# gmh14/tssplat

Measured on AMD Instinct MI355X. Metric: tetrahedra/sec (energy fwd+bwd), higher is better.
Workload: dtype f32

## Files before the change

### include/tssplat_amd.h

```cpp
#ifndef TSSPLAT_AMD_H
#define TSSPLAT_AMD_H

#include <stdint.h>

#ifdef __cplusplus
extern "C" {
#endif

typedef struct tsamd_handle tsamd_handle;

typedef enum tsamd_status {
    TSAMD_OK = 0,
    TSAMD_ERR_INVALID_ARGUMENT = 1,
    TSAMD_ERR_BAD_MESH = 2,
    TSAMD_ERR_NO_DEVICE = 3,
    TSAMD_ERR_HIP = 4,
    TSAMD_ERR_IO = 5,
    TSAMD_ERR_TILING = 6,
    TSAMD_ERR_HOST_ONLY = 7
} tsamd_status;

typedef struct tsamd_options {
    int32_t struct_size;
    int32_t device;
// ... 11 lines not shown

typedef struct tsamd_plan_info {
    int64_t n_vertices, n_tets;
    int64_t n_tiles;
    int64_t n_components;
    int64_t total_slots;
    int64_t total_tile_vertices;
    int64_t shared_vertex_copies;
    int64_t finish_vertices;
    int64_t device_bytes;
    int32_t max_slots, max_tile_vertices, block_threads, lds_bytes;
    int32_t slots_per_thread;
    int32_t n_planes;
} tsamd_plan_info;

typedef struct tsamd_tile_view {
    int32_t n_slots, n_owned, s_pad, n_verts, n_excl;
    int64_t stage_off;
    int32_t n_rows;
    int32_t rec_base;
    const uint32_t *planes;
    const uint16_t *row_start;
    const int32_t *gvid;
    const int32_t *vdst;
    const int32_t *slot_tet;
    const float *rest;
} tsamd_tile_view;

const char *tsamd_last_error(void);
const char *tsamd_version(void);
#define TSAMD_ABI_VERSION 3
int32_t tsamd_abi_version(void);

int tsamd_create(const float *rest_xyz, int64_t n_vertices, const int32_t *tets, int64_t n_tets,
                 const tsamd_options *options, tsamd_handle **out);
int tsamd_create_from_veg(const char *path, const tsamd_options *options, tsamd_handle **out);
int tsamd_create_with_operator(const float *rest_xyz, int64_t n_vertices, const int32_t *tets, int64_t n_tets,
                               const int64_t *op_rowptr, const int32_t *op_col, const double *op_val,
                               const tsamd_options *options, tsamd_handle **out);
void tsamd_destroy(tsamd_handle *h);

int64_t tsamd_num_vertices(const tsamd_handle *h);
int64_t tsamd_num_tets(const tsamd_handle *h);
int tsamd_get_plan_info(const tsamd_handle *h, tsamd_plan_info *out);
int tsamd_get_tile(const tsamd_handle *h, int64_t tile, tsamd_tile_view *out);
int tsamd_get_finish_lists(const tsamd_handle *h, int64_t *n_finish, const int32_t **vid,
                           const int32_t **off, const int32_t **idx);
int tsamd_get_adjacency(const tsamd_handle *h, const int32_t **nbr);

int tsamd_forward(tsamd_handle *h, const float *x_dev, float c1, float c2, int order,
                  void *stream, float *energy_dev);
int tsamd_backward(tsamd_handle *h, const float *x_dev, const float *grad_out_dev, float c1, float c2,
                   int order, void *stream, float *grad_dev);
int tsamd_forward_backward(tsamd_handle *h, const float *x_dev, const float *grad_out_dev, float c1,
                           float c2, int order, void *stream, float *energy_dev, float *grad_dev);
int tsamd_evaluate_dev_coef(tsamd_handle *h, const float *x_dev, const float *grad_out_dev, const float *coef_dev,
                            int order, void *stream, float *energy_dev, float *grad_dev);
typedef struct tsamd_graph tsamd_graph;
int tsamd_graph_create(tsamd_handle *h, const float *x_dev, const float *grad_out_dev, int order, float *energy_dev,
// ... 101 lines not shown
```

### tssplat_amd/_capi.py

```python
from __future__ import annotations

import ctypes as C
import os

from . import _build

_lib = None


class TsamdError(RuntimeError):

    def __init__(self, code: int, message: str):
        super().__init__(f"tssplat_amd error {code}: {message}")
        self.code = code


class Options(C.Structure):
    _fields_ = [
        ("struct_size", C.c_int32),
        ("device", C.c_int32),
        ("lds_budget_bytes", C.c_int32),
        ("max_threads", C.c_int32),
        ("target_owned", C.c_int32),
        ("lane_search_sweeps", C.c_int32),
# ... 7 lines not shown


class PlanInfo(C.Structure):
    _fields_ = [
        ("n_vertices", C.c_int64), ("n_tets", C.c_int64), ("n_tiles", C.c_int64),
        ("n_components", C.c_int64), ("total_slots", C.c_int64), ("total_tile_vertices", C.c_int64),
        ("shared_vertex_copies", C.c_int64), ("finish_vertices", C.c_int64), ("device_bytes", C.c_int64),
        ("max_slots", C.c_int32), ("max_tile_vertices", C.c_int32), ("block_threads", C.c_int32),
        ("lds_bytes", C.c_int32), ("slots_per_thread", C.c_int32), ("n_planes", C.c_int32),
    ]

    def as_dict(self) -> dict:
        return {k: int(getattr(self, k)) for k, _ in self._fields_}


class TileView(C.Structure):
    _fields_ = [
        ("n_slots", C.c_int32), ("n_owned", C.c_int32), ("s_pad", C.c_int32), ("n_verts", C.c_int32),
        ("n_excl", C.c_int32), ("stage_off", C.c_int64), ("n_rows", C.c_int32), ("rec_base", C.c_int32),
        ("planes", C.POINTER(C.c_uint32)), ("row_start", C.POINTER(C.c_uint16)),
        ("gvid", C.POINTER(C.c_int32)), ("vdst", C.POINTER(C.c_int32)), ("slot_tet", C.POINTER(C.c_int32)), ("rest", C.POINTER(C.c_float)),
    ]


ABI_VERSION = 3

SIGNATURES = {
    "tsamd_last_error": (C.c_char_p, []),
    "tsamd_version": (C.c_char_p, []),
    "tsamd_abi_version": (C.c_int32, []),
    "tsamd_create": (C.c_int, [C.c_void_p, C.c_int64, C.c_void_p, C.c_int64, C.POINTER(Options), C.POINTER(C.c_void_p)]),
    "tsamd_create_with_operator": (C.c_int, [C.c_void_p, C.c_int64, C.c_void_p, C.c_int64, C.c_void_p, C.c_void_p, C.c_void_p,
                                             C.POINTER(Options), C.POINTER(C.c_void_p)]),
    "tsamd_create_from_veg": (C.c_int, [C.c_char_p, C.POINTER(Options), C.POINTER(C.c_void_p)]),
    "tsamd_destroy": (None, [C.c_void_p]),
    "tsamd_num_vertices": (C.c_int64, [C.c_void_p]),
    "tsamd_num_tets": (C.c_int64, [C.c_void_p]),
    "tsamd_get_plan_info": (C.c_int, [C.c_void_p, C.POINTER(PlanInfo)]),
    "tsamd_get_tile": (C.c_int, [C.c_void_p, C.c_int64, C.POINTER(TileView)]),
    "tsamd_get_finish_lists": (C.c_int, [C.c_void_p, C.POINTER(C.c_int64), C.POINTER(C.POINTER(C.c_int32)),
                                         C.POINTER(C.POINTER(C.c_int32)), C.POINTER(C.POINTER(C.c_int32))]),
    "tsamd_get_adjacency": (C.c_int, [C.c_void_p, C.POINTER(C.POINTER(C.c_int32))]),
    "tsamd_forward": (C.c_int, [C.c_void_p, C.c_void_p, C.c_float, C.c_float, C.c_int, C.c_void_p, C.c_void_p]),
    "tsamd_backward": (C.c_int, [C.c_void_p, C.c_void_p, C.c_void_p, C.c_float, C.c_float, C.c_int, C.c_void_p,
                                 C.c_void_p]),
    "tsamd_forward_backward": (C.c_int, [C.c_void_p, C.c_void_p, C.c_void_p, C.c_float, C.c_float, C.c_int,
                                         C.c_void_p, C.c_void_p, C.c_void_p]),
    "tsamd_evaluate_dev_coef": (C.c_int, [C.c_void_p, C.c_void_p, C.c_void_p, C.c_void_p, C.c_int, C.c_void_p, C.c_void_p,
                                          C.c_void_p]),
    "tsamd_graph_create": (C.c_int, [C.c_void_p, C.c_void_p, C.c_void_p, C.c_int, C.c_void_p, C.c_void_p, C.POINTER(C.c_void_p)]),
    "tsamd_graph_launch": (C.c_int, [C.c_void_p, C.c_float, C.c_float, C.c_void_p]),
    "tsamd_graph_launch_to": (C.c_int, [C.c_void_p, C.c_float, C.c_float, C.c_void_p, C.c_void_p, C.c_void_p]),
    "tsamd_graph_destroy": (None, [C.c_void_p]),
# ... 134 lines not shown
```

### tssplat_amd/csrc/capi.cpp

```cpp
#include "../../include/tssplat_amd.h"

#include <hip/hip_runtime_api.h>

#include <algorithm>
#include <cmath>
#include <cstdio>
#include <cstdlib>
#include <cstring>
#include <new>
#include <string>
#include <thread>
#include <vector>

#include "capi_common.h"
#include "kernels.h"
#include "plan.h"

namespace {

thread_local std::string g_err;

int fail(int code, const std::string &msg)
{
    g_err = msg;
// ... 323 lines not shown
    out->n_components = P.n_components;
    out->total_slots = P.total_slots;
    out->total_tile_vertices = P.total_tile_verts;
    out->shared_vertex_copies = P.n_stage;
    out->finish_vertices = int64_t(P.fin_vid.size());
    out->device_bytes = h->device_bytes;
    out->max_slots = P.max_slots;
    out->max_tile_vertices = P.max_verts;
    out->block_threads = P.block_threads;
    out->lds_bytes = P.lds_bytes;
    out->slots_per_thread = P.spt;
    out->n_planes = P.n_planes;
    return TSAMD_OK;
}

int tsamd_get_tile(const tsamd_handle *h, int64_t tile, tsamd_tile_view *out)
{
    if (!h || !out) return fail(TSAMD_ERR_INVALID_ARGUMENT, "null argument");
    const tsamd::Plan &P = h->plan;
    if (tile < 0 || tile >= int64_t(P.tiles.size())) return fail(TSAMD_ERR_INVALID_ARGUMENT, "tile out of range");
    const tsamd::TileDesc &d = P.tiles[size_t(tile)];
    out->n_slots = d.n_slots;
    out->n_owned = d.n_owned;
    out->s_pad = d.s_pad;
    out->n_verts = d.n_verts;
    out->n_excl = d.n_excl;
    out->stage_off = d.stage_off;
    out->n_rows = d.n_rows;
    out->rec_base = d.rec_base;
    out->planes = P.blob.data() + d.blob_off / 4;
// ... 254 lines not shown
```

### tssplat_amd/csrc/partition.cpp

```cpp
#include "partition.h"

#include <algorithm>
#include <cmath>

namespace tsamd {
namespace {

constexpr int kLloydIters = 12;
constexpr int kLloydFull = 4;
constexpr int kCandidates = 8;
constexpr int kImproveSweeps = 6;
constexpr int kConnectProbe = 512;
constexpr int64_t kMaxIncidence = int64_t(1) << 23;

inline int64_t copies(int64_t c) { return (c + kMaxRank - 1) / kMaxRank; }

struct Part {
    const Limits &lim;
    int64_t cnt = 0, nv = 0, k = 0;
    std::vector<int32_t> nb;
    std::vector<int32_t> lv;
    std::vector<double> x;
    std::vector<int32_t> part;
    std::vector<int64_t> owned, slots, verts;
    std::vector<int32_t> inc;
    std::vector<int32_t> mark, queue;
    int32_t stamp = 0;

    explicit Part(const Limits &l) : lim(l) {}

    int64_t cost(int64_t p) const { return kPartSlotWeight * slots[size_t(p)] + verts[size_t(p)]; }
    bool fits(int64_t p) const { return lim.fits(slots[size_t(p)], verts[size_t(p)]); }

    void seed(int32_t *idx, int64_t n, int64_t kk, int32_t &next)
    {
        if (kk <= 1) {
            for (int64_t i = 0; i < n; ++i) part[size_t(idx[i])] = next;
            ++next;
            return;
        }
        double lo[3], hi[3];
        for (int d = 0; d < 3; ++d) {
            lo[d] = std::numeric_limits<double>::max();
            hi[d] = -std::numeric_limits<double>::max();
        }
        for (int64_t i = 0; i < n; ++i)
// ... 147 lines not shown
                        pc[np] = pr;
                        nn[np++] = 0;
                    }
                    ++nn[j];
                }
                if (np == 0) continue;
                int j = 0;
                for (int i = 1; i < np; ++i)
                    if (nn[i] > nn[j] || (nn[i] == nn[j] && pc[i] < pc[j])) j = i;
                part[size_t(e)] = pc[j];
                --left;
            }
        }
    }

    void add_slot(int32_t p, int32_t e)
    {
        ++slots[size_t(p)];
        for (int a = 0; a < 4; ++a) {
            int32_t &c = inc[size_t(p) * size_t(nv) + size_t(lv[4 * size_t(e) + a])];
            if (c % kMaxRank == 0) ++verts[size_t(p)];
            ++c;
        }
    }
    void remove_slot(int32_t p, int32_t e)
    {
        --slots[size_t(p)];
        for (int a = 0; a < 4; ++a) {
            int32_t &c = inc[size_t(p) * size_t(nv) + size_t(lv[4 * size_t(e) + a])];
            --c;
            if (c % kMaxRank == 0) --verts[size_t(p)];
        }
    }
    void build_state()
    {
        owned.assign(size_t(k), 0);
        slots.assign(size_t(k), 0);
        verts.assign(size_t(k), 0);
        inc.assign(size_t(k) * size_t(nv), 0);
        for (int64_t q = 0; q < cnt; ++q) {
            const int32_t pq = part[size_t(q)];
            ++owned[size_t(pq)];
            add_slot(pq, int32_t(q));
            int32_t seen[4];
            int ns = 0;
            for (int f = 0; f < 4; ++f) {
                const int32_t r = nb[4 * size_t(q) + f];
                if (r < 0) continue;
                const int32_t pr = part[size_t(r)];
                if (pr == pq || std::find(seen, seen + ns, pr) != seen + ns) continue;
                seen[ns++] = pr;
                add_slot(pr, int32_t(q));
            }
        }
// ... 28 lines not shown
            if (q < 0 || part[size_t(q)] == A || !first_of(e, f)) continue;
            if (in_cell(q, A) == 1) out[n++] = q;
        }
        return n;
    }
    int entering(int32_t e, int32_t B, int32_t *out) const
    {
        int n = 0;
        for (int f = 0; f < 4; ++f) {
            const int32_t q = nb[4 * size_t(e) + f];
            if (q < 0 || part[size_t(q)] == B || !first_of(e, f)) continue;
            if (in_cell(q, B) == 0) out[n++] = q;
        }
        return n;
    }
    int64_t vert_delta(int32_t p, const int32_t *t, int n, int sign) const
    {
        int32_t vs[20], ds[20];
        int m = 0;
        for (int i = 0; i < n; ++i)
            for (int a = 0; a < 4; ++a) {
                const int32_t v = lv[4 * size_t(t[i]) + a];
                int j = int(std::find(vs, vs + m, v) - vs);
                if (j == m) {
                    vs[m] = v;
                    ds[m++] = 0;
                }
                ds[j] += sign;
            }
        int64_t d = 0;
        for (int j = 0; j < m; ++j) {
            const int32_t c = inc[size_t(p) * size_t(nv) + size_t(vs[j])];
            d += copies(c + ds[j]) - copies(c);
        }
        return d;
    }
    struct Move {
        int32_t e = -1, B = -1;
        int64_t dcost = 0, key = 0;
        int nl = 0, ne = 0;
        int32_t gone[5], en[4];
        int64_t dsA = 0, dvA = 0, dsB = 0, dvB = 0;
    };
    bool evaluate(int32_t e, int32_t B, Move &mv) const
    {
        const int32_t A = part[size_t(e)];
        mv.e = e;
        mv.B = B;
        mv.nl = leaving(e, A, mv.gone);
        mv.ne = entering(e, B, mv.en);
        mv.dsA = -mv.nl;
        mv.dsB = mv.ne;
        mv.dvB = vert_delta(B, mv.en, mv.ne, +1);
        if (!lim.fits(slots[size_t(B)] + mv.dsB, verts[size_t(B)] + mv.dvB)) return false;
        mv.dvA = vert_delta(A, mv.gone, mv.nl, -1);
        mv.dcost = kPartSlotWeight * (mv.dsA + mv.dsB) + mv.dvA + mv.dvB;
        return true;
    }
    void apply(const Move &mv)
    {
        const int32_t A = part[size_t(mv.e)];
        for (int i = 0; i < mv.nl; ++i) remove_slot(A, mv.gone[i]);
        for (int i = 0; i < mv.ne; ++i) add_slot(mv.B, mv.en[i]);
        part[size_t(mv.e)] = mv.B;
        --owned[size_t(A)];
        ++owned[size_t(mv.B)];
    }
    bool stays_connected(int32_t e)
    {
        const int32_t A = part[size_t(e)];
        int32_t want[4];
// ... 40 lines not shown
        for (int64_t A = 0; A < k; ++A) {
            if (fits(A)) continue;
            members.clear();
            for (int64_t e = 0; e < cnt; ++e)
                if (part[size_t(e)] == A) members.push_back(int32_t(e));
            while (!fits(A)) {
                if (owned[size_t(A)] <= 1) return false;
                Move best, mv;
                bool have = false;
                for (int32_t e : members) {
                    if (part[size_t(e)] != A) continue;
                    int32_t oc[4];
                    const int no = other_cells(e, oc);
                    for (int j = 0; j < no; ++j) {
                        if (!evaluate(e, oc[j], mv)) continue;
                        mv.key = mv.dcost + kPartSlotWeight * mv.dsA + mv.dvA;
                        if (have && mv.key >= best.key) continue;
                        if (!stays_connected(e)) break;
                        best = mv;
                        have = true;
                    }
                }
                if (!have) return false;
                apply(best);
            }
        }
        return true;
    }

    void improve()
    {
        for (int sweep = 0; sweep < kImproveSweeps; ++sweep) {
            int64_t moved = 0;
            for (int64_t e = 0; e < cnt; ++e) {
                const int32_t A = part[size_t(e)];
                if (owned[size_t(A)] <= 1) continue;
                int32_t oc[4];
                const int no = other_cells(int32_t(e), oc);
                Move best, mv;
                bool have = false;
                for (int j = 0; j < no; ++j) {
                    if (!evaluate(int32_t(e), oc[j], mv) || mv.dcost >= 0) continue;
                    if (have && mv.dcost >= best.dcost) continue;
                    best = mv;
                    have = true;
                }
                if (have && stays_connected(int32_t(e))) {
                    apply(best);
                    ++moved;
                }
            }
            if (moved == 0) break;
        }
    }
};

}

bool partition_component(const Mesh &M, const Limits &lim, const float *cen, const int32_t *ids, int64_t cnt,
                         int64_t k_first, int64_t k_last, Scratch &S, std::vector<std::vector<int32_t>> &parts,
                         int64_t &cost)
{
    parts.clear();
    cost = 0;
    k_first = std::max<int64_t>(2, k_first);
    k_last = std::min(k_last, cnt);
    if (k_first > k_last) return false;
    Part P(lim);
    P.cnt = cnt;
    P.nb.resize(4 * size_t(cnt));
    P.lv.resize(4 * size_t(cnt));
    P.x.resize(3 * size_t(cnt));
    const int32_t st = S.next();
    for (int64_t i = 0; i < cnt; ++i) {
        S.tet_stamp[size_t(ids[i])] = st;
        S.tet_slot[size_t(ids[i])] = int32_t(i);
    }
    for (int64_t i = 0; i < cnt; ++i) {
        const int64_t g = ids[i];
        for (int f = 0; f < 4; ++f) {
            const int32_t q = M.nbr[4 * g + f];
            P.nb[4 * size_t(i) + f] = q >= 0 && S.tet_stamp[size_t(q)] == st ? S.tet_slot[size_t(q)] : -1;
            const int32_t v = M.tets[4 * g + f];
            if (S.vert_stamp[size_t(v)] != st) {
                S.vert_stamp[size_t(v)] = st;
                S.vert_local[size_t(v)] = int32_t(P.nv++);
            }
            P.lv[4 * size_t(i) + f] = S.vert_local[size_t(v)];
        }
        for (int d = 0; d < 3; ++d) P.x[3 * size_t(i) + d] = cen[3 * size_t(g) + d];
    }
    if (k_last * P.nv > kMaxIncidence) return false;
    P.mark.assign(size_t(cnt), 0);
    std::vector<int32_t> idx(static_cast<size_t>(cnt));
    for (int64_t k = k_first; k <= k_last; ++k) {
        P.k = k;
        P.part.assign(size_t(cnt), 0);
        for (int64_t i = 0; i < cnt; ++i) idx[size_t(i)] = int32_t(i);
        int32_t next = 0;
        P.seed(idx.data(), cnt, k, next);
        P.lloyd();
        P.connect();
        P.build_state();
        if (!P.repair()) continue;
        P.improve();
        std::vector<int64_t> at(size_t(k), -1);
        for (int64_t p = 0; p < k; ++p)
            if (P.owned[size_t(p)] > 0) {
                at[size_t(p)] = int64_t(parts.size());
                parts.emplace_back();
                parts.back().reserve(size_t(P.owned[size_t(p)]));
                cost += P.cost(p);
            }
        for (int64_t i = 0; i < cnt; ++i) parts[size_t(at[size_t(P.part[size_t(i)])])].push_back(ids[i]);
        return true;
    }
    return false;
}

}
```

### tssplat_amd/csrc/partition.h

```cpp
#pragma once

#include "plan.h"

#include <cstdint>
#include <limits>
#include <vector>

namespace tsamd {

struct Scratch {
    std::vector<int32_t> tet_stamp, tet_slot, vert_stamp, vert_local;
    int32_t stamp = 0;
    void init(int64_t m, int64_t n)
    {
        if (int64_t(tet_stamp.size()) != m) {
            tet_stamp.assign(size_t(m), 0);
            tet_slot.assign(size_t(m), 0);
        }
        if (int64_t(vert_stamp.size()) != n) {
            vert_stamp.assign(size_t(n), 0);
            vert_local.assign(size_t(n), 0);
        }
    }
    int32_t next()
// ... 18 lines not shown
        const int64_t sp = (n_slots + pad_unit - 1) / pad_unit * pad_unit;
        return sp <= max_spad && n_verts <= kMaxTileVerts && tile_lds_bytes(sp, n_verts, rebuild) <= budget;
    }
};

struct Mesh {
    const float *rest;
    const int32_t *tets;
    const int32_t *nbr;
    int64_t n, m;
};

void measure(const Mesh &M, const int32_t *owned, int64_t cnt, Scratch &S, int64_t &n_slots, int64_t &n_verts,
             std::vector<int32_t> *halo_out = nullptr);

constexpr int64_t kPartSlotWeight = 3;

bool partition_component(const Mesh &M, const Limits &lim, const float *cen, const int32_t *ids, int64_t cnt,
                         int64_t k_first, int64_t k_last, Scratch &S, std::vector<std::vector<int32_t>> &parts,
                         int64_t &cost);

}
```

### tssplat_amd/csrc/plan.cpp

```cpp
#include "plan.h"

#include "conflict_opt.h"
#include "partition.h"

#include <algorithm>
#include <atomic>
#include <cmath>
#include <cstdio>
#include <cstdlib>
#include <cstring>
#include <fstream>
#include <functional>
#include <limits>
#include <numeric>
#include <sstream>
#include <chrono>
#include <thread>

namespace tsamd {
namespace {

struct StageTimer {
    bool on = std::getenv("TSAMD_PLAN_TIMING") != nullptr;
    std::chrono::steady_clock::time_point t0 = std::chrono::steady_clock::now();
// ... 513 lines not shown
            sp.failed = false;
            if (!done) sp.split(ids, cnt, (cnt + target - 1) / target);
            if (sp.rc) {
                first_rc.store(sp.rc);
                bool expected = false;
                if (err_set.compare_exchange_strong(expected, true)) split_err = local_err;
            }
        }
    });
    if (first_rc.load()) {
        err = split_err;
        return first_rc.load();
    }

    timer.lap("bisection");
    std::vector<int64_t> rcb_slots(groups.size(), 0), rcb_cost(groups.size(), 0), rcb_lds(groups.size(), 0);
    parallel_chunks(int64_t(groups.size()), 16, nthreads, [&](int64_t b, int64_t e, int w) {
        Scratch &S = get_scratch(w);
        for (int64_t g = b; g < e; ++g)
            for (const auto &l : group_tiles[size_t(g)]) {
                int64_t ns, nv;
                measure(M, l.data(), int64_t(l.size()), S, ns, nv);
                rcb_slots[size_t(g)] += ns;
                rcb_cost[size_t(g)] += kPartSlotWeight * ns + nv;
                const int64_t sp = (ns + lim.pad_unit - 1) / lim.pad_unit * lim.pad_unit;
                rcb_lds[size_t(g)] = std::max(rcb_lds[size_t(g)], tile_lds_bytes(sp, nv, rebuild));
            }
    });
    Limits cell_lim = lim;
    cell_lim.budget = 0;
    for (int64_t l : rcb_lds) cell_lim.budget = std::max(cell_lim.budget, std::min(lim.budget, l));
    std::atomic<int64_t> n_cut{0}, n_refined{0};
    parallel_chunks(int64_t(groups.size()), 1, nthreads, [&](int64_t b, int64_t e, int w) {
        Scratch &S = get_scratch(w);
        std::vector<std::vector<int32_t>> parts;
        for (int64_t g = b; g < e; ++g) {
            if (!group_fitted[size_t(g)]) continue;
            const Group &G = groups[size_t(g)];
            const int32_t *ids = comp_tets.data() + comp_start[G.cb];
            const int64_t cnt = comp_start[G.ce] - comp_start[G.cb];
            auto &leaves = group_tiles[size_t(g)];
            const int64_t k_rcb = int64_t(leaves.size());
            n_cut.fetch_add(1, std::memory_order_relaxed);
            const int64_t k_lo = (rcb_slots[size_t(g)] + s_cap - 1) / s_cap;
            int64_t cost;
            if (!partition_component(M, cell_lim, cen.data(), ids, cnt, k_lo, std::min(k_rcb, k_lo + 3), S, parts, cost)) continue;
            if (int64_t(parts.size()) > k_rcb || (int64_t(parts.size()) == k_rcb && cost >= rcb_cost[size_t(g)])) continue;
            n_refined.fetch_add(1, std::memory_order_relaxed);
            leaves.clear();
            std::string unused_err;
            Splitter sp{M, lim, cen, S, leaves, unused_err};
            for (auto &part : parts) sp.emit(part.data(), int64_t(part.size()));
        }
    });
    if (timer.on)
        std::fprintf(stderr, "[plan] partition: %lld cut components, %lld refined, %lld keep the bisection\n", (long long)n_cut.load(),
                     (long long)n_refined.load(), (long long)(n_cut.load() - n_refined.load()));
    timer.lap("partition (cells + refinement)");
    std::vector<std::vector<int32_t>> tiles_owned;
    for (auto &gt : group_tiles)
        for (auto &t : gt) tiles_owned.push_back(std::move(t));
    group_tiles.clear();
    const int64_t T = int64_t(tiles_owned.size());

    std::vector<std::vector<int32_t>> tile_halo(static_cast<size_t>(T)), tile_verts(static_cast<size_t>(T)), tile_vdeg(static_cast<size_t>(T));
    std::vector<std::atomic<int32_t>> vcount(static_cast<size_t>(n));
    for (auto &a : vcount) a.store(0, std::memory_order_relaxed);
    parallel_chunks(T, 4, nthreads, [&](int64_t b, int64_t e, int w) {
        Scratch &S = get_scratch(w);
        std::vector<int32_t> uniq, cnt;
        std::vector<std::pair<int32_t, int32_t>> key;
        for (int64_t t = b; t < e; ++t) {
// ... 501 lines not shown
```

### tssplat_amd/csrc/plan.h

```cpp
#pragma once

#include <cstdint>
#include <memory>
#include <string>
#include <utility>
#include <vector>

#ifdef __HIPCC__
#define TSAMD_HOST_DEVICE __host__ __device__
#else
#define TSAMD_HOST_DEVICE
#endif

namespace tsamd {

struct PlanOptions {
    int lds_budget = 0;
    int max_threads = 0;
    int target_owned = 0;
    int num_threads = 0;
    int conflict_aware = 1;
    int lane_search_sweeps = 2;
    int rebuild_dminv = 0;
    int slots_per_lane = 0;
// ... 79 lines not shown
using RawVector = std::vector<T, DefaultInitAllocator<T>>;

struct Plan {
    int64_t n = 0, m = 0;
    int64_t n_components = 0;
    std::vector<int32_t> nbr;
    std::vector<TileDesc> tiles;
    RawVector<uint32_t> blob;
    RawVector<int32_t> gvid;
    RawVector<int32_t> vdst;
    RawVector<int32_t> slot_tet;
    std::vector<int64_t> slot_base;
    std::vector<int32_t> fin_vid, fin_off, fin_idx;
    int64_t n_stage = 0;
    int64_t total_slots = 0, total_tile_verts = 0;
    int32_t max_slots = 0, max_verts = 0, block_threads = 64, lds_bytes = 0, spt = kSlotsPerLane;
    int32_t n_planes = kPlanes;
    int32_t vert_stride = 64;
    std::vector<float> op_diag;
    std::vector<float> op_w;
};

struct ElementOperatorCSR {
    const int64_t *rowptr;
    const int32_t *col;
    const double *val;
};

int build_plan(const float *rest, int64_t n, const int32_t *tets, int64_t m, const PlanOptions &opt,
               Plan &plan, std::string &err, const ElementOperatorCSR *op = nullptr);
// ... 8 lines not shown
```

### tssplat_amd/tet_spheres_ext.py

```python
from __future__ import annotations

import contextlib
import ctypes as C
import os
import sys

import numpy as np
import torch

from . import _capi

__all__ = ["TetSpheres", "forward", "backward", "random_x", "grad_limit"]

_lib = _capi.load()
CPU_ENERGY = os.environ.get("TSSPLAT_AMD_CPU_ENERGY", "0") == "1"
REBUILD_DMINV = {"1": 1, "2": 2}.get(os.environ.get("TSSPLAT_AMD_REBUILD_DMINV", "0"), 0)
print("initializing")


_raw_stream = getattr(torch._C, "_cuda_getCurrentRawStream", None)


def _stream_ptr(device: torch.device) -> int:
    if _raw_stream is not None and device.index is not None:
# ... 82 lines not shown

    def __del__(self):
        try:
            self.close()
        except Exception:
            pass

    def _handle(self):
        if not self._h.value:
            raise RuntimeError("TetSpheres object is empty (construction failed or it was closed)")
        return self._h

    def plan_info(self) -> dict:
        info = _capi.PlanInfo()
        _capi.check(_lib.tsamd_get_plan_info(self._handle(), C.byref(info)))
        return info.as_dict()

    def set_timing(self, enable: bool) -> None:
        _capi.check(_lib.tsamd_set_timing(self._handle(), int(enable)))

    def get_timing(self) -> tuple[float, float, int]:
        a, b, n = C.c_double(), C.c_double(), C.c_int64()
        _capi.check(_lib.tsamd_get_timing(self._handle(), C.byref(a), C.byref(b), C.byref(n)))
        return a.value, b.value, n.value

    def energy_terms(self) -> tuple[float, float]:
        out = (C.c_double * 2)()
        _capi.check(_lib.tsamd_read_energy_terms(self._handle(), _stream_ptr(self.device), out))
        return float(out[0]), float(out[1])


# ... 80 lines not shown
```

Baseline: 58.65 billion.

## Refine tile partition with FM passes, staged-row cost and template reuse

Replaces greedy improvement sweeps in the mesh tile partitioner with Fiduccia-Mattheyses style passes using a priority queue and rollback to the best prefix. The cost now penalises vertices staged across multiple tiles (shared-copy rows) instead of per-tile vertex counts, plus a region-growing reseed step. Identical component shapes are detected by hash and geometry check so one cut is reused as a template. The aim is fewer halo slots and staged rows, which cuts global traffic and the finish reduction in the energy kernel, at the cost of longer plan build time. Adds a partition info query API.

After: 60.24 billion (median of 6 runs). 2.7% higher.

```diff
diff --git a/include/tssplat_amd.h b/include/tssplat_amd.h
--- a/include/tssplat_amd.h
+++ b/include/tssplat_amd.h
@@ -49,6 +49,19 @@
     int32_t n_planes;
 } tsamd_plan_info;
 
+typedef struct tsamd_partition_info {
+    int64_t owned_tets;
+    int64_t halo_slots;
+    int64_t staged_rows;
+    int64_t n_tiles;
+    int64_t tile_capacity;
+    int64_t min_tiles;
+    int64_t cut_components;
+    int64_t bisection_components;
+    int64_t cut_templates;
+    double mean_fill, max_fill;
+} tsamd_partition_info;
+
 typedef struct tsamd_tile_view {
     int32_t n_slots, n_owned, s_pad, n_verts, n_excl;
     int64_t stage_off;
@@ -78,6 +91,7 @@
 int64_t tsamd_num_vertices(const tsamd_handle *h);
 int64_t tsamd_num_tets(const tsamd_handle *h);
 int tsamd_get_plan_info(const tsamd_handle *h, tsamd_plan_info *out);
+int tsamd_get_partition_info(const tsamd_handle *h, tsamd_partition_info *out);
 int tsamd_get_tile(const tsamd_handle *h, int64_t tile, tsamd_tile_view *out);
 int tsamd_get_finish_lists(const tsamd_handle *h, int64_t *n_finish, const int32_t **vid,
                            const int32_t **off, const int32_t **idx);
diff --git a/tssplat_amd/_capi.py b/tssplat_amd/_capi.py
--- a/tssplat_amd/_capi.py
+++ b/tssplat_amd/_capi.py
@@ -45,6 +45,14 @@
         return {k: int(getattr(self, k)) for k, _ in self._fields_}
 
 
+class PartitionInfo(C.Structure):
+    _fields_ = [
+        ("owned_tets", C.c_int64), ("halo_slots", C.c_int64), ("staged_rows", C.c_int64), ("n_tiles", C.c_int64),
+        ("tile_capacity", C.c_int64), ("min_tiles", C.c_int64), ("cut_components", C.c_int64),
+        ("bisection_components", C.c_int64), ("cut_templates", C.c_int64), ("mean_fill", C.c_double), ("max_fill", C.c_double),
+    ]
+
+
 class TileView(C.Structure):
     _fields_ = [
         ("n_slots", C.c_int32), ("n_owned", C.c_int32), ("s_pad", C.c_int32), ("n_verts", C.c_int32),
@@ -68,6 +76,7 @@
     "tsamd_num_vertices": (C.c_int64, [C.c_void_p]),
     "tsamd_num_tets": (C.c_int64, [C.c_void_p]),
     "tsamd_get_plan_info": (C.c_int, [C.c_void_p, C.POINTER(PlanInfo)]),
+    "tsamd_get_partition_info": (C.c_int, [C.c_void_p, C.POINTER(PartitionInfo)]),
     "tsamd_get_tile": (C.c_int, [C.c_void_p, C.c_int64, C.POINTER(TileView)]),
     "tsamd_get_finish_lists": (C.c_int, [C.c_void_p, C.POINTER(C.c_int64), C.POINTER(C.POINTER(C.c_int32)),
                                          C.POINTER(C.POINTER(C.c_int32)), C.POINTER(C.POINTER(C.c_int32))]),
diff --git a/tssplat_amd/csrc/capi.cpp b/tssplat_amd/csrc/capi.cpp
--- a/tssplat_amd/csrc/capi.cpp
+++ b/tssplat_amd/csrc/capi.cpp
@@ -361,6 +361,27 @@
     return TSAMD_OK;
 }
 
+int tsamd_get_partition_info(const tsamd_handle *h, tsamd_partition_info *out)
+{
+    if (!h || !out) return fail(TSAMD_ERR_INVALID_ARGUMENT, "null argument");
+    const tsamd::Plan &P = h->plan;
+    std::memset(out, 0, sizeof(*out));
+    out->owned_tets = P.m;
+    out->halo_slots = P.total_slots - P.m;
+    out->staged_rows = P.n_stage;
+    out->n_tiles = int64_t(P.tiles.size());
+    out->tile_capacity = int64_t(P.block_threads) * P.spt;
+    out->min_tiles = out->tile_capacity > 0 ? (P.total_slots + out->tile_capacity - 1) / out->tile_capacity : 0;
+    out->cut_components = P.n_cut_components;
+    out->bisection_components = P.n_bisection_components;
+    out->cut_templates = P.n_cut_templates;
+    if (out->n_tiles > 0 && out->tile_capacity > 0) {
+        out->mean_fill = double(P.total_slots) / (double(out->n_tiles) * double(out->tile_capacity));
+        out->max_fill = double(P.max_slots) / double(out->tile_capacity);
+    }
+    return TSAMD_OK;
+}
+
 int tsamd_get_tile(const tsamd_handle *h, int64_t tile, tsamd_tile_view *out)
 {
     if (!h || !out) return fail(TSAMD_ERR_INVALID_ARGUMENT, "null argument");
diff --git a/tssplat_amd/csrc/partition.cpp b/tssplat_amd/csrc/partition.cpp
--- a/tssplat_amd/csrc/partition.cpp
+++ b/tssplat_amd/csrc/partition.cpp
@@ -2,6 +2,8 @@
 
 #include <algorithm>
 #include <cmath>
+#include <set>
+#include <utility>
 
 namespace tsamd {
 namespace {
@@ -9,7 +11,9 @@
 constexpr int kLloydIters = 12;
 constexpr int kLloydFull = 4;
 constexpr int kCandidates = 8;
-constexpr int kImproveSweeps = 6;
+constexpr int kGrowRounds = 6;
+constexpr int kFmPasses = 8;
+constexpr int kFmStall = 3000;
 constexpr int kConnectProbe = 512;
 constexpr int64_t kMaxIncidence = int64_t(1) << 23;
 
@@ -24,12 +28,20 @@
     std::vector<int32_t> part;
     std::vector<int64_t> owned, slots, verts;
     std::vector<int32_t> inc;
+    std::vector<int32_t> tot;
+    int64_t rows = 0;
     std::vector<int32_t> mark, queue;
     int32_t stamp = 0;
 
     explicit Part(const Limits &l) : lim(l) {}
 
-    int64_t cost(int64_t p) const { return kPartSlotWeight * slots[size_t(p)] + verts[size_t(p)]; }
+    static int64_t staged(int64_t c) { return c > 1 ? c : 0; }
+    int64_t total_slots() const
+    {
+        int64_t s = 0;
+        for (int64_t p = 0; p < k; ++p) s += slots[size_t(p)];
+        return s;
+    }
     bool fits(int64_t p) const { return lim.fits(slots[size_t(p)], verts[size_t(p)]); }
 
     void seed(int32_t *idx, int64_t n, int64_t kk, int32_t &next)
@@ -207,12 +219,79 @@
         }
     }
 
+    void grow(int rounds)
+    {
+        const size_t K = size_t(k);
+        std::vector<double> c(3 * K);
+        std::vector<int64_t> n_in(K);
+        std::vector<int32_t> centre(K), claimed(static_cast<size_t>(cnt));
+        std::vector<std::vector<int32_t>> fifo(K);
+        std::vector<size_t> head(K);
+        for (int it = 0; it < rounds; ++it) {
+            std::fill(c.begin(), c.end(), 0.0);
+            std::fill(n_in.begin(), n_in.end(), 0);
+            for (int64_t e = 0; e < cnt; ++e) {
+                const int32_t p = part[size_t(e)];
+                ++n_in[size_t(p)];
+                for (int d = 0; d < 3; ++d) c[3 * size_t(p) + d] += x[3 * size_t(e) + d];
+            }
+            std::vector<double> best(K, std::numeric_limits<double>::max());
+            std::fill(centre.begin(), centre.end(), -1);
+            for (int64_t e = 0; e < cnt; ++e) {
+                const int32_t p = part[size_t(e)];
+                double d2 = 0.0;
+                for (int d = 0; d < 3; ++d) {
+                    const double t = x[3 * size_t(e) + d] - c[3 * size_t(p) + d] / double(n_in[size_t(p)]);
+                    d2 += t * t;
+                }
+                if (d2 < best[size_t(p)]) {
+                    best[size_t(p)] = d2;
+                    centre[size_t(p)] = int32_t(e);
+                }
+            }
+            std::fill(claimed.begin(), claimed.end(), -1);
+            std::fill(n_in.begin(), n_in.end(), 0);
+            for (size_t p = 0; p < K; ++p) {
+                fifo[p].clear();
+                head[p] = 0;
+                if (centre[p] >= 0) fifo[p].push_back(centre[p]);
+            }
+            for (int64_t left = cnt; left > 0;) {
+                int64_t p = -1;
+                for (size_t q = 0; q < K; ++q) {
+                    while (head[q] < fifo[q].size() && claimed[size_t(fifo[q][head[q]])] >= 0) ++head[q];
+                    if (head[q] < fifo[q].size() && (p < 0 || n_in[q] < n_in[size_t(p)])) p = int64_t(q);
+                }
+                if (p < 0) break;
+                const int32_t e = fifo[size_t(p)][head[size_t(p)]++];
+                claimed[size_t(e)] = int32_t(p);
+                ++n_in[size_t(p)];
+                --left;
+                for (int f = 0; f < 4; ++f) {
+                    const int32_t r = nb[4 * size_t(e) + f];
+                    if (r >= 0 && claimed[size_t(r)] < 0) fifo[size_t(p)].push_back(r);
+                }
+            }
+            for (int64_t e = 0; e < cnt; ++e)
+                if (claimed[size_t(e)] >= 0) part[size_t(e)] = claimed[size_t(e)];
+        }
+    }
+
+    void copy_changed(int32_t v, int d)
+    {
+        rows -= staged(tot[size_t(v)]);
+        tot[size_t(v)] += d;
+        rows += staged(tot[size_t(v)]);
+    }
     void add_slot(int32_t p, int32_t e)
     {
         ++slots[size_t(p)];
         for (int a = 0; a < 4; ++a) {
             int32_t &c = inc[size_t(p) * size_t(nv) + size_t(lv[4 * size_t(e) + a])];
-            if (c % kMaxRank == 0) ++verts[size_t(p)];
+            if (c % kMaxRank == 0) {
+                ++verts[size_t(p)];
+                copy_changed(lv[4 * size_t(e) + a], +1);
+            }
             ++c;
         }
     }
@@ -222,7 +301,10 @@
         for (int a = 0; a < 4; ++a) {
             int32_t &c = inc[size_t(p) * size_t(nv) + size_t(lv[4 * size_t(e) + a])];
             --c;
-            if (c % kMaxRank == 0) --verts[size_t(p)];
+            if (c % kMaxRank == 0) {
+                --verts[size_t(p)];
+                copy_changed(lv[4 * size_t(e) + a], -1);
+            }
         }
     }
     void build_state()
@@ -231,6 +313,8 @@
         slots.assign(size_t(k), 0);
         verts.assign(size_t(k), 0);
         inc.assign(size_t(k) * size_t(nv), 0);
+        tot.assign(size_t(nv), 0);
+        rows = 0;
         for (int64_t q = 0; q < cnt; ++q) {
             const int32_t pq = part[size_t(q)];
             ++owned[size_t(pq)];
@@ -289,27 +373,6 @@
         }
         return n;
     }
-    int64_t vert_delta(int32_t p, const int32_t *t, int n, int sign) const
-    {
-        int32_t vs[20], ds[20];
-        int m = 0;
-        for (int i = 0; i < n; ++i)
-            for (int a = 0; a < 4; ++a) {
-                const int32_t v = lv[4 * size_t(t[i]) + a];
-                int j = int(std::find(vs, vs + m, v) - vs);
-                if (j == m) {
-                    vs[m] = v;
-                    ds[m++] = 0;
-                }
-                ds[j] += sign;
-            }
-        int64_t d = 0;
-        for (int j = 0; j < m; ++j) {
-            const int32_t c = inc[size_t(p) * size_t(nv) + size_t(vs[j])];
-            d += copies(c + ds[j]) - copies(c);
-        }
-        return d;
-    }
     struct Move {
         int32_t e = -1, B = -1;
         int64_t dcost = 0, key = 0;
@@ -317,7 +380,7 @@
         int32_t gone[5], en[4];
         int64_t dsA = 0, dvA = 0, dsB = 0, dvB = 0;
     };
-    bool evaluate(int32_t e, int32_t B, Move &mv) const
+    bool evaluate(int32_t e, int32_t B, Move &mv, bool check = true) const
     {
         const int32_t A = part[size_t(e)];
         mv.e = e;
@@ -326,10 +389,34 @@
         mv.ne = entering(e, B, mv.en);
         mv.dsA = -mv.nl;
         mv.dsB = mv.ne;
-        mv.dvB = vert_delta(B, mv.en, mv.ne, +1);
-        if (!lim.fits(slots[size_t(B)] + mv.dsB, verts[size_t(B)] + mv.dvB)) return false;
-        mv.dvA = vert_delta(A, mv.gone, mv.nl, -1);
-        mv.dcost = kPartSlotWeight * (mv.dsA + mv.dsB) + mv.dvA + mv.dvB;
+        int32_t vs[36], dA[36], dB[36];
+        int m = 0;
+        auto note = [&](int32_t t, int32_t *d, int sign) {
+            for (int a = 0; a < 4; ++a) {
+                const int32_t v = lv[4 * size_t(t) + a];
+                int j = int(std::find(vs, vs + m, v) - vs);
+                if (j == m) {
+                    vs[m] = v;
+                    dA[m] = dB[m] = 0;
+                    ++m;
+                }
+                d[j] += sign;
+            }
+        };
+        for (int i = 0; i < mv.nl; ++i) note(mv.gone[i], dA, -1);
+        for (int i = 0; i < mv.ne; ++i) note(mv.en[i], dB, +1);
+        mv.dvA = mv.dvB = 0;
+        int64_t drows = 0;
+        for (int j = 0; j < m; ++j) {
+            const int32_t cA = inc[size_t(A) * size_t(nv) + size_t(vs[j])], cB = inc[size_t(B) * size_t(nv) + size_t(vs[j])];
+            const int64_t a = copies(cA + dA[j]) - copies(cA), b = copies(cB + dB[j]) - copies(cB);
+            mv.dvA += a;
+            mv.dvB += b;
+            const int64_t t = tot[size_t(vs[j])];
+            drows += staged(t + a + b) - staged(t);
+        }
+        if (check && !lim.fits(slots[size_t(B)] + mv.dsB, verts[size_t(B)] + mv.dvB)) return false;
+        mv.dcost = kPartSlotWeight * (mv.dsA + mv.dsB) + kPartRowWeight * drows;
         return true;
     }
     void apply(const Move &mv)
@@ -400,7 +487,7 @@
                     const int no = other_cells(e, oc);
                     for (int j = 0; j < no; ++j) {
                         if (!evaluate(e, oc[j], mv)) continue;
-                        mv.key = mv.dcost + kPartSlotWeight * mv.dsA + mv.dvA;
+                        mv.key = mv.dcost + kPartSlotWeight * mv.dsA + kPartRowWeight * mv.dvA;
                         if (have && mv.key >= best.key) continue;
                         if (!stays_connected(e)) break;
                         best = mv;
@@ -414,29 +501,137 @@
         return true;
     }
 
+    bool best_move(int32_t e, Move &best) const
+    {
+        if (owned[size_t(part[size_t(e)])] <= 1) return false;
+        int32_t oc[4];
+        const int no = other_cells(e, oc);
+        Move mv;
+        bool have = false;
+        for (int j = 0; j < no; ++j) {
+            if (!evaluate(e, oc[j], mv)) continue;
+            if (have && (mv.dcost > best.dcost || (mv.dcost == best.dcost && mv.B > best.B))) continue;
+            best = mv;
+            have = true;
+        }
+        return have;
+    }
+    std::set<std::pair<int64_t, int32_t>> fm_queue;
+    std::vector<int64_t> fm_key;
+    std::vector<uint8_t> fm_queued, fm_locked;
+    void fm_drop(int32_t e)
+    {
+        if (!fm_queued[size_t(e)]) return;
+        fm_queue.erase({fm_key[size_t(e)], e});
+        fm_queued[size_t(e)] = 0;
+    }
+    void fm_refresh(int32_t e)
+    {
+        fm_drop(e);
+        Move mv;
+        if (fm_locked[size_t(e)] || !best_move(e, mv)) return;
+        fm_key[size_t(e)] = mv.dcost;
+        fm_queued[size_t(e)] = 1;
+        fm_queue.insert({mv.dcost, e});
+    }
+    bool fm_pass()
+    {
+        fm_queue.clear();
+        fm_key.assign(size_t(cnt), 0);
+        fm_queued.assign(size_t(cnt), 0);
+        fm_locked.assign(size_t(cnt), 0);
+        for (int64_t e = 0; e < cnt; ++e) fm_refresh(int32_t(e));
+        std::vector<std::pair<int32_t, int32_t>> done;
+        int64_t cum = 0, best = 0;
+        size_t best_len = 0;
+        while (!fm_queue.empty() && done.size() - best_len < size_t(kFmStall)) {
+            const int32_t e = fm_queue.begin()->second;
+            Move mv;
+            if (!best_move(e, mv)) {
+                fm_drop(e);
+                continue;
+            }
+            if (mv.dcost != fm_key[size_t(e)]) {
+                fm_queue.erase(fm_queue.begin());
+                fm_key[size_t(e)] = mv.dcost;
+                fm_queue.insert({mv.dcost, e});
+                continue;
+            }
+            fm_drop(e);
+            if (!stays_connected(e)) continue;
+            const int32_t A = part[size_t(e)];
+            apply(mv);
+            fm_locked[size_t(e)] = 1;
+            done.push_back({e, A});
+            cum += mv.dcost;
+            if (cum < best) {
+                best = cum;
+                best_len = done.size();
+            }
+            for (int f = 0; f < 4; ++f) {
+                const int32_t q = nb[4 * size_t(e) + f];
+                if (q < 0) continue;
+                fm_refresh(q);
+                for (int g = 0; g < 4; ++g) {
+                    const int32_t r = nb[4 * size_t(q) + g];
+                    if (r >= 0 && r != e) fm_refresh(r);
+                }
+            }
+        }
+        while (done.size() > best_len) {
+            Move mv;
+            evaluate(done.back().first, done.back().second, mv, false);
+            apply(mv);
+            done.pop_back();
+        }
+        return best < 0;
+    }
     void improve()
     {
-        for (int sweep = 0; sweep < kImproveSweeps; ++sweep) {
-            int64_t moved = 0;
+        for (int pass = 0; pass < kFmPasses; ++pass)
+            if (!fm_pass()) break;
+    }
+
+    void seed_spread()
+    {
+        double mean[3] = {0.0, 0.0, 0.0};
+        for (int64_t e = 0; e < cnt; ++e)
+            for (int d = 0; d < 3; ++d) mean[d] += x[3 * size_t(e) + d];
+        for (int d = 0; d < 3; ++d) mean[d] /= double(cnt);
+        std::vector<double> d2(size_t(cnt), std::numeric_limits<double>::max());
+        auto dist2 = [&](int64_t e, const double *c) {
+            double s = 0.0;
+            for (int d = 0; d < 3; ++d) {
+                const double t = x[3 * size_t(e) + d] - c[d];
+                s += t * t;
+            }
+            return s;
+        };
+        int64_t far = 0;
+        double far_d = -1.0;
+        for (int64_t e = 0; e < cnt; ++e) {
+            const double d = dist2(e, mean);
+            if (d > far_d) {
+                far_d = d;
+                far = e;
+            }
+        }
+        for (int64_t p = 0; p < k; ++p) {
+            const double *c = &x[3 * size_t(far)];
+            int64_t next_far = 0;
+            double next_d = -1.0;
             for (int64_t e = 0; e < cnt; ++e) {
-                const int32_t A = part[size_t(e)];
-                if (owned[size_t(A)] <= 1) continue;
-                int32_t oc[4];
-                const int no = other_cells(int32_t(e), oc);
-                Move best, mv;
-                bool have = false;
-                for (int j = 0; j < no; ++j) {
-                    if (!evaluate(int32_t(e), oc[j], mv) || mv.dcost >= 0) continue;
-                    if (have && mv.dcost >= best.dcost) continue;
-                    best = mv;
-                    have = true;
-                }
-                if (have && stays_connected(int32_t(e))) {
-                    apply(best);
-                    ++moved;
-                }
-            }
-            if (moved == 0) break;
+                const double d = dist2(e, c);
+                if (d < d2[size_t(e)]) {
+                    d2[size_t(e)] = d;
+                    part[size_t(e)] = int32_t(p);
+                }
+                if (d2[size_t(e)] > next_d) {
+                    next_d = d2[size_t(e)];
+                    next_far = e;
+                }
+            }
+            far = next_far;
         }
     }
 };
@@ -444,11 +639,11 @@
 }
 
 bool partition_component(const Mesh &M, const Limits &lim, const float *cen, const int32_t *ids, int64_t cnt,
-                         int64_t k_first, int64_t k_last, Scratch &S, std::vector<std::vector<int32_t>> &parts,
-                         int64_t &cost)
+                         const std::vector<std::vector<int32_t>> &incumbent, int64_t k_first, int64_t k_last, int64_t slot_cap,
+                         Scratch &S, std::vector<std::vector<int32_t>> &parts, CutStats &before, CutStats &after)
 {
     parts.clear();
-    cost = 0;
+    before = after = CutStats();
     k_first = std::max<int64_t>(2, k_first);
     k_last = std::min(k_last, cnt);
     if (k_first > k_last) return false;
@@ -476,32 +671,70 @@
         }
         for (int d = 0; d < 3; ++d) P.x[3 * size_t(i) + d] = cen[3 * size_t(g) + d];
     }
-    if (k_last * P.nv > kMaxIncidence) return false;
+    if (std::max<int64_t>(k_last, int64_t(incumbent.size())) * P.nv > kMaxIncidence) return false;
     P.mark.assign(size_t(cnt), 0);
-    std::vector<int32_t> idx(static_cast<size_t>(cnt));
-    for (int64_t k = k_first; k <= k_last; ++k) {
+    P.k = int64_t(incumbent.size());
+    P.part.assign(size_t(cnt), 0);
+    for (size_t p = 0; p < incumbent.size(); ++p)
+        for (int32_t g : incumbent[p]) P.part[size_t(S.tet_slot[size_t(g)])] = int32_t(p);
+    P.build_state();
+    before.parts = P.k;
+    before.slots = P.total_slots();
+    before.rows = P.rows;
+    std::vector<int32_t> idx(static_cast<size_t>(cnt)), best_part;
+    int64_t best_k = 0;
+    after = before;
+    auto try_k = [&](int64_t k) {
         P.k = k;
-        P.part.assign(size_t(cnt), 0);
-        for (int64_t i = 0; i < cnt; ++i) idx[size_t(i)] = int32_t(i);
-        int32_t next = 0;
-        P.seed(idx.data(), cnt, k, next);
-        P.lloyd();
-        P.connect();
-        P.build_state();
-        if (!P.repair()) continue;
-        P.improve();
-        std::vector<int64_t> at(size_t(k), -1);
-        for (int64_t p = 0; p < k; ++p)
-            if (P.owned[size_t(p)] > 0) {
-                at[size_t(p)] = int64_t(parts.size());
-                parts.emplace_back();
-                parts.back().reserve(size_t(P.owned[size_t(p)]));
-                cost += P.cost(p);
-            }
-        for (int64_t i = 0; i < cnt; ++i) parts[size_t(at[size_t(P.part[size_t(i)])])].push_back(ids[i]);
-        return true;
-    }
-    return false;
+        bool any = false;
+        for (int grown = 0; grown < 2; ++grown) {
+            bool fitted = false;
+            for (int spread = 0; spread < 2 && !fitted; ++spread) {
+                P.part.assign(size_t(cnt), 0);
+                if (spread) {
+                    P.seed_spread();
+                } else {
+                    for (int64_t i = 0; i < cnt; ++i) idx[size_t(i)] = int32_t(i);
+                    int32_t next = 0;
+                    P.seed(idx.data(), cnt, k, next);
+                }
+                P.lloyd();
+                P.connect();
+                if (grown) P.grow(kGrowRounds);
+                P.build_state();
+                fitted = P.repair();
+            }
+            if (!fitted) continue;
+            any = true;
+            P.improve();
+            CutStats now;
+            for (int64_t p = 0; p < k; ++p) now.parts += P.owned[size_t(p)] > 0;
+            now.slots = P.total_slots();
+            now.rows = P.rows;
+            if (now.cost() >= after.cost()) continue;
+            after = now;
+            best_part = P.part;
+            best_k = k;
+        }
+        return any;
+    };
+    int fitted_ks = 0;
+    for (int64_t k = k_first; k <= k_last && fitted_ks < 2; ++k) fitted_ks += try_k(k) ? 1 : 0;
+    for (int64_t k = k_first - 1; k >= 2 && best_k == k + 1 && (after.slots + slot_cap - 1) / slot_cap <= k; --k) try_k(k);
+    if (best_k == 0 || after.cost() * kPartMinSavingDen > before.cost() * (kPartMinSavingDen - 1)) {
+        after = before;
+        return false;
+    }
+    std::vector<int64_t> at(size_t(best_k), -1);
+    for (int64_t i = 0; i < cnt; ++i) {
+        int64_t &a = at[size_t(best_part[size_t(i)])];
+        if (a < 0) {
+            a = int64_t(parts.size());
+            parts.emplace_back();
+        }
+        parts[size_t(a)].push_back(ids[i]);
+    }
+    return true;
 }
 
 }
diff --git a/tssplat_amd/csrc/partition.h b/tssplat_amd/csrc/partition.h
--- a/tssplat_amd/csrc/partition.h
+++ b/tssplat_amd/csrc/partition.h
@@ -56,10 +56,18 @@
 void measure(const Mesh &M, const int32_t *owned, int64_t cnt, Scratch &S, int64_t &n_slots, int64_t &n_verts,
              std::vector<int32_t> *halo_out = nullptr);
 
-constexpr int64_t kPartSlotWeight = 3;
+constexpr int64_t kPartSlotWeight = 7;
+constexpr int64_t kPartRowWeight = 2;
+
+constexpr int64_t kPartMinSavingDen = 40;
+
+struct CutStats {
+    int64_t parts = 0, slots = 0, rows = 0;
+    int64_t cost() const { return kPartSlotWeight * slots + kPartRowWeight * rows; }
+};
 
 bool partition_component(const Mesh &M, const Limits &lim, const float *cen, const int32_t *ids, int64_t cnt,
-                         int64_t k_first, int64_t k_last, Scratch &S, std::vector<std::vector<int32_t>> &parts,
-                         int64_t &cost);
+                         const std::vector<std::vector<int32_t>> &incumbent, int64_t k_first, int64_t k_last, int64_t slot_cap,
+                         Scratch &S, std::vector<std::vector<int32_t>> &parts, CutStats &before, CutStats &after);
 
 }
diff --git a/tssplat_amd/csrc/plan.cpp b/tssplat_amd/csrc/plan.cpp
--- a/tssplat_amd/csrc/plan.cpp
+++ b/tssplat_amd/csrc/plan.cpp
@@ -551,15 +551,13 @@
     }
 
     timer.lap("bisection");
-    std::vector<int64_t> rcb_slots(groups.size(), 0), rcb_cost(groups.size(), 0), rcb_lds(groups.size(), 0);
+    std::vector<int64_t> rcb_lds(groups.size(), 0);
     parallel_chunks(int64_t(groups.size()), 16, nthreads, [&](int64_t b, int64_t e, int w) {
         Scratch &S = get_scratch(w);
         for (int64_t g = b; g < e; ++g)
             for (const auto &l : group_tiles[size_t(g)]) {
                 int64_t ns, nv;
                 measure(M, l.data(), int64_t(l.size()), S, ns, nv);
-                rcb_slots[size_t(g)] += ns;
-                rcb_cost[size_t(g)] += kPartSlotWeight * ns + nv;
                 const int64_t sp = (ns + lim.pad_unit - 1) / lim.pad_unit * lim.pad_unit;
                 rcb_lds[size_t(g)] = std::max(rcb_lds[size_t(g)], tile_lds_bytes(sp, nv, rebuild));
             }
@@ -567,32 +565,135 @@
     Limits cell_lim = lim;
     cell_lim.budget = 0;
     for (int64_t l : rcb_lds) cell_lim.budget = std::max(cell_lim.budget, std::min(lim.budget, l));
-    std::atomic<int64_t> n_cut{0}, n_refined{0};
+    struct Shape {
+        int32_t vbase = 0;
+        uint64_t hash = 0;
+        double lo[3], hi[3];
+    };
+    std::vector<Shape> shape(groups.size());
+    std::vector<int64_t> model(groups.size(), -1);
+    auto comp_ids = [&](int64_t g, int64_t &cnt) -> int32_t * {
+        cnt = comp_start[groups[size_t(g)].ce] - comp_start[groups[size_t(g)].cb];
+        return comp_tets.data() + comp_start[groups[size_t(g)].cb];
+    };
+    parallel_chunks(int64_t(groups.size()), 1, nthreads, [&](int64_t b, int64_t e, int) {
+        for (int64_t g = b; g < e; ++g) {
+            if (!group_fitted[size_t(g)]) continue;
+            int64_t cnt;
+            int32_t *ids = comp_ids(g, cnt);
+            std::sort(ids, ids + cnt);
+            Shape &sh = shape[size_t(g)];
+            sh.vbase = std::numeric_limits<int32_t>::max();
+            for (int d = 0; d < 3; ++d) {
+                sh.lo[d] = std::numeric_limits<double>::max();
+                sh.hi[d] = -std::numeric_limits<double>::max();
+            }
+            for (int64_t i = 0; i < cnt; ++i)
+                for (int a = 0; a < 4; ++a) {
+                    const int32_t v = tets[4 * int64_t(ids[i]) + a];
+                    sh.vbase = std::min(sh.vbase, v);
+                    for (int d = 0; d < 3; ++d) {
+                        sh.lo[d] = std::min(sh.lo[d], double(rest[3 * size_t(v) + d]));
+                        sh.hi[d] = std::max(sh.hi[d], double(rest[3 * size_t(v) + d]));
+                    }
+                }
+            uint64_t h = 1469598103934665603ull ^ uint64_t(cnt);
+            for (int64_t i = 0; i < cnt; ++i) {
+                h = (h ^ uint64_t(ids[i] - ids[0])) * 1099511628211ull;
+                for (int a = 0; a < 4; ++a) h = (h ^ uint64_t(tets[4 * int64_t(ids[i]) + a] - sh.vbase)) * 1099511628211ull;
+            }
+            sh.hash = h;
+        }
+    });
+    {
+        std::vector<std::pair<uint64_t, int64_t>> by_hash;
+        for (size_t g = 0; g < groups.size(); ++g)
+            if (group_fitted[g]) by_hash.push_back({shape[g].hash, int64_t(g)});
+        std::sort(by_hash.begin(), by_hash.end());
+        for (size_t i = 0; i < by_hash.size(); ++i)
+            model[size_t(by_hash[i].second)] = i > 0 && by_hash[i - 1].first == by_hash[i].first ? model[size_t(by_hash[i - 1].second)] : by_hash[i].second;
+    }
+    constexpr double kSimilarTol = 1e-4;
+    parallel_chunks(int64_t(groups.size()), 1, nthreads, [&](int64_t b, int64_t e, int) {
+        for (int64_t g = b; g < e; ++g) {
+            const int64_t r = model[size_t(g)];
+            if (r < 0 || r == g) continue;
+            int64_t cnt, cnt_r;
+            const int32_t *ids = comp_ids(g, cnt), *ids_r = comp_ids(r, cnt_r);
+            const Shape &sg = shape[size_t(g)], &sr = shape[size_t(r)];
+            bool same = cnt == cnt_r;
+            double ext_g = 0.0, ext_r = 0.0;
+            for (int d = 0; d < 3; ++d) {
+                ext_g = std::max(ext_g, sg.hi[d] - sg.lo[d]);
+                ext_r = std::max(ext_r, sr.hi[d] - sr.lo[d]);
+            }
+            same = same && ext_g > 0.0 && ext_r > 0.0;
+            const double scale = same ? ext_g / ext_r : 1.0;
+            for (int64_t i = 0; i < cnt && same; ++i) {
+                same = ids[i] - ids[0] == ids_r[i] - ids_r[0];
+                for (int a = 0; a < 4 && same; ++a) {
+                    const int32_t v = tets[4 * int64_t(ids[i]) + a], vr = tets[4 * int64_t(ids_r[i]) + a];
+                    same = v - sg.vbase == vr - sr.vbase;
+                    for (int d = 0; d < 3 && same; ++d)
+                        same = std::fabs((double(rest[3 * size_t(v) + d]) - sg.lo[d]) - scale * (double(rest[3 * size_t(vr) + d]) - sr.lo[d])) <= kSimilarTol * ext_g;
+                }
+            }
+            if (!same) model[size_t(g)] = g;
+        }
+    });
+    std::vector<std::vector<std::vector<int32_t>>> cut(groups.size());
+    std::vector<uint8_t> refined(groups.size(), 0);
     parallel_chunks(int64_t(groups.size()), 1, nthreads, [&](int64_t b, int64_t e, int w) {
         Scratch &S = get_scratch(w);
-        std::vector<std::vector<int32_t>> parts;
         for (int64_t g = b; g < e; ++g) {
-            if (!group_fitted[size_t(g)]) continue;
-            const Group &G = groups[size_t(g)];
-            const int32_t *ids = comp_tets.data() + comp_start[G.cb];
-            const int64_t cnt = comp_start[G.ce] - comp_start[G.cb];
+            if (model[size_t(g)] != g) continue;
+            int64_t cnt;
+            const int32_t *ids = comp_ids(g, cnt);
+            const auto &leaves = group_tiles[size_t(g)];
+            const int64_t k_rcb = int64_t(leaves.size());
+            int64_t rcb_slots = 0;
+            for (const auto &l : leaves) {
+                int64_t ns, nv;
+                measure(M, l.data(), int64_t(l.size()), S, ns, nv);
+                rcb_slots += ns;
+            }
+            const int64_t k_lo = (rcb_slots + s_cap - 1) / s_cap;
+            CutStats before, after;
+            refined[size_t(g)] = partition_component(M, cell_lim, cen.data(), ids, cnt, leaves, k_lo, std::min(k_rcb, k_lo + 3), s_cap, S, cut[size_t(g)], before, after) ? 1 : 0;
+        }
+    });
+    int64_t n_cut = 0, n_refined = 0, n_models = 0;
+    for (size_t g = 0; g < groups.size(); ++g) {
+        if (model[g] < 0) continue;
+        ++n_cut;
+        n_models += model[g] == int64_t(g);
+        n_refined += refined[size_t(model[g])];
+    }
+    parallel_chunks(int64_t(groups.size()), 1, nthreads, [&](int64_t b, int64_t e, int w) {
+        Scratch &S = get_scratch(w);
+        std::vector<int32_t> part;
+        for (int64_t g = b; g < e; ++g) {
+            const int64_t r = model[size_t(g)];
+            if (r < 0 || !refined[size_t(r)]) continue;
+            int64_t cnt, cnt_r;
+            const int32_t *ids = comp_ids(g, cnt), *ids_r = comp_ids(r, cnt_r);
             auto &leaves = group_tiles[size_t(g)];
-            const int64_t k_rcb = int64_t(leaves.size());
-            n_cut.fetch_add(1, std::memory_order_relaxed);
-            const int64_t k_lo = (rcb_slots[size_t(g)] + s_cap - 1) / s_cap;
-            int64_t cost;
-            if (!partition_component(M, cell_lim, cen.data(), ids, cnt, k_lo, std::min(k_rcb, k_lo + 3), S, parts, cost)) continue;
-            if (int64_t(parts.size()) > k_rcb || (int64_t(parts.size()) == k_rcb && cost >= rcb_cost[size_t(g)])) continue;
-            n_refined.fetch_add(1, std::memory_order_relaxed);
             leaves.clear();
             std::string unused_err;
             Splitter sp{M, lim, cen, S, leaves, unused_err};
-            for (auto &part : parts) sp.emit(part.data(), int64_t(part.size()));
-        }
-    });
+            for (const auto &c : cut[size_t(r)]) {
+                part.resize(c.size());
+                for (size_t i = 0; i < c.size(); ++i) part[i] = c[i] - ids_r[0] + ids[0];
+                sp.emit(part.data(), int64_t(part.size()));
+            }
+        }
+    });
+    P.n_cut_components = n_cut;
+    P.n_bisection_components = n_cut - n_refined;
+    P.n_cut_templates = n_models;
     if (timer.on)
-        std::fprintf(stderr, "[plan] partition: %lld cut components, %lld refined, %lld keep the bisection\n", (long long)n_cut.load(),
-                     (long long)n_refined.load(), (long long)(n_cut.load() - n_refined.load()));
+        std::fprintf(stderr, "[plan] partition: %lld cut components, %lld refined, %lld keep the bisection (%lld cut themselves)\n", (long long)n_cut,
+                     (long long)n_refined, (long long)(n_cut - n_refined), (long long)n_models);
     timer.lap("partition (cells + refinement)");
     std::vector<std::vector<int32_t>> tiles_owned;
     for (auto &gt : group_tiles)
diff --git a/tssplat_amd/csrc/plan.h b/tssplat_amd/csrc/plan.h
--- a/tssplat_amd/csrc/plan.h
+++ b/tssplat_amd/csrc/plan.h
@@ -117,6 +117,7 @@
     std::vector<int32_t> fin_vid, fin_off, fin_idx;
     int64_t n_stage = 0;
     int64_t total_slots = 0, total_tile_verts = 0;
+    int64_t n_cut_components = 0, n_bisection_components = 0, n_cut_templates = 0;
     int32_t max_slots = 0, max_verts = 0, block_threads = 64, lds_bytes = 0, spt = kSlotsPerLane;
     int32_t n_planes = kPlanes;
     int32_t vert_stride = 64;
diff --git a/tssplat_amd/tet_spheres_ext.py b/tssplat_amd/tet_spheres_ext.py
--- a/tssplat_amd/tet_spheres_ext.py
+++ b/tssplat_amd/tet_spheres_ext.py
@@ -120,7 +120,13 @@
     def plan_info(self) -> dict:
         info = _capi.PlanInfo()
         _capi.check(_lib.tsamd_get_plan_info(self._handle(), C.byref(info)))
-        return info.as_dict()
+        out = info.as_dict()
+        cut = _capi.PartitionInfo()
+        _capi.check(_lib.tsamd_get_partition_info(self._handle(), C.byref(cut)))
+        for k, _ in cut._fields_:
+            if k != "n_tiles":
+                out[k] = getattr(cut, k)
+        return out
 
     def set_timing(self, enable: bool) -> None:
         _capi.check(_lib.tsamd_set_timing(self._handle(), int(enable)))
```
